# Duy1230/Map-Reduced-Approach-for-Vietnamese-Long-Document-Summarization

Measured on AMD Instinct MI355X. Metric: map-phase chunks/sec (2k-tok chunk, 256-tok summary) at 1/2/4/8 MI355X, higher is better.
Workload: dtype f16

## Files before the change

### include/mapsum.h

```cpp
#ifndef MAPSUM_H
#define MAPSUM_H

#include <stddef.h>
#include <stdint.h>

#ifdef __cplusplus
extern "C" {
#endif

#define MS_ABI_VERSION 3

#define MS_OK 0
#define MS_EIO -5
#define MS_ENOMEM -12
#define MS_EBUSY -16
#define MS_EINVAL -22
#define MS_ENOSPC -28

#define MS_FINISH_EOS 1
#define MS_FINISH_LENGTH 2
#define MS_FINISH_ERROR 3

#define MS_FLAG_IGNORE_EOS 1u

// ... 30 lines not shown
  int32_t eos_ids[8];
} ms_config;

typedef struct ms_result {
  uint64_t tag;
  const int32_t* ids;
  int32_t n_ids;
  int32_t finish_reason;
  int32_t n_prompt;
  int32_t _pad;
} ms_result;

typedef struct ms_stats {
  int64_t prefill_tokens;
  int64_t decode_tokens;
  int64_t prefill_passes, decode_steps;
  int64_t finished;
  double prefill_ms, decode_ms;
  double kernel_ms[8];
  int64_t kernel_launches[8];
  int64_t decode_kv_tokens;
  int64_t graphs_built;
  int64_t persist_fallbacks;
  int64_t persist_steps;
} ms_stats;

typedef struct ms_engine ms_engine;

int ms_create(const ms_config* cfg, ms_engine** out);
int ms_destroy(ms_engine* e);
const char* ms_last_error(const ms_engine* e);

int ms_enable_qk_norm(ms_engine* e);

int ms_load_weight(ms_engine* e, int32_t tensor, int32_t layer, const uint16_t* host_f16,
                   int64_t n_elems);
int ms_init_synthetic(ms_engine* e, uint64_t seed, float std, float norm_jitter);

#define MS_GGML_Q8_0 8
#define MS_GGML_Q4_K 12
#define MS_GGML_Q5_K 13
#define MS_GGML_Q6_K 14
int ms_load_weight_q(ms_engine* e, int32_t tensor, int32_t layer, int32_t ggml_type,
                     const void* host_blocks, int64_t n_bytes);
int ms_init_synthetic_q(ms_engine* e, uint64_t seed, float scale, float norm_jitter);
int ms_init_synthetic_q8_0(ms_engine* e, uint64_t seed, float scale, float norm_jitter);
int ms_init_synthetic_q5_k_m(ms_engine* e, uint64_t seed, float scale, float norm_jitter);

int ms_weight_regions(const ms_engine* e, void** ptrs, int64_t* bytes, int32_t cap);
int ms_quant_manifest(const ms_engine* e, int32_t* triples, int32_t cap);
int ms_declare_weight_q(ms_engine* e, int32_t tensor, int32_t layer, int32_t ggml_type);

int ms_submit(ms_engine* e, const int32_t* ids, int32_t n, int32_t num_predict,
              uint32_t flags, uint64_t tag);
#define MS_SAMPLE_MAX_TOPK 256
#define MS_SAMPLE_MAX_WINDOW 256
typedef struct ms_sampling {
  float temperature;
  int32_t top_k;
  float top_p;
  float min_p;
  float repeat_penalty;
  int32_t repeat_last_n;
  uint64_t seed;
} ms_sampling;
int ms_submit_sampled(ms_engine* e, const int32_t* ids, int32_t n, int32_t num_predict,
                      uint32_t flags, uint64_t tag, const ms_sampling* sp);
int ms_set_eos_ids(ms_engine* e, const int32_t* ids, int32_t n);
int ms_step(ms_engine* e);
int ms_poll(ms_engine* e, ms_result* out, int32_t cap);
int ms_pending(const ms_engine* e);
int ms_get_stats(const ms_engine* e, ms_stats* out);
int ms_reset_stats(ms_engine* e);
int ms_set_profiling(ms_engine* e, uint32_t class_mask);
int ms_trace_push(const char* name);
int ms_trace_pop(void);
int ms_synchronize(ms_engine* e);
int ms_set_persist(ms_engine* e, int32_t on);
#define MS_DBG_KPOOL 0
#define MS_DBG_VPOOL 1
#define MS_DBG_DECODE_LOGITS 2
#define MS_DBG_DECODE_X 3
#define MS_DBG_PREFILL_LOGITS 4
int ms_debug_read(ms_engine* e, int32_t which, int64_t offset, void* host, int64_t bytes);
int ms_debug_pk_stamps(uint64_t* out, int32_t n);
int ms_debug_a2_stamps(uint64_t* out, int32_t n);
int ms_debug_gemv_stamps(uint64_t* out, int32_t n);

int ms_forward(ms_engine* e, const int32_t* ids, int32_t n, int32_t n_layers_run,
               float* hidden_out, float* logits_out);
int ms_forward_packed(ms_engine* e, const int32_t* ids, const int32_t* lens, int32_t n_seqs,
                      int32_t n_layers_run, float* hidden_out, float* logits_out);
int ms_submit_forced(ms_engine* e, const int32_t* ids, int32_t n, const int32_t* forced,
                     int32_t n_forced, int32_t num_predict, uint32_t flags, uint64_t tag);

#define MS_EPI_STORE_F16 0
#define MS_EPI_ADD_F32 1
#define MS_EPI_SWIGLU 2
#define MS_EPI_STORE_F32 3
#define MS_EPI_ARGMAX 5
int ms_op_gemm(const void* A, const void* W, void* out, int32_t M, int32_t N, int32_t K,
               int32_t ldo, int32_t epilogue, void* stream);
int ms_op_gemm_resid(const void* A, const void* W, float* x, void* xg_out, const void* gamma, float* ssq_out,
                     int32_t M, int32_t N, int32_t K, void* stream);
int ms_gemm_resid_tiles(int32_t M, int32_t N);
int ms_set_gemm_variant(int32_t variant);
#define MS_GEMV_ORDER_DEFAULT (-1)
int ms_set_gemv_order(int32_t order);
int ms_set_qgemv_gs(int32_t on);
int ms_set_attn_tuning(int32_t combine_grp, int32_t order);
int ms_set_dgemm_kh(int32_t kh);
int ms_set_dgemm_wn(int32_t wn);
int64_t ms_op_gemv_workspace(int32_t M, int32_t N, int32_t K);
int ms_op_gemv(const void* X, const void* W, void* out, int32_t M, int32_t N, int32_t K,
               int32_t ldo, int32_t epilogue, void* workspace, void* stream);
int ms_op_gemv_tuned(const void* X, const void* W, void* out, int32_t M, int32_t N, int32_t K,
                     int32_t ldo, int32_t epilogue, void* workspace, int32_t waves, void* stream);
int ms_op_gemv_strided(const void* X, const void* W, void* out, int32_t M, int32_t N, int32_t K,
                       int32_t ldk, int32_t ldo, int32_t epilogue, void* stream);
int ms_op_gemv_resid(const void* X, const void* W, float* x, void* xg_out, const void* gamma,
                     float* ssq_out, int32_t M, int32_t N, int32_t K, int32_t rt, void* stream);
int ms_op_set_row_scale(const float* ssq, int32_t tiles, int32_t hidden, float eps);
int ms_op_dgemm(const void* X, const void* W, void* out, int32_t M, int32_t N, int32_t K, int32_t S,
                int32_t ldo, int32_t epilogue, void* stream);
int ms_op_gemv_split(const void* X, const void* W, float* slabs, int32_t M, int32_t N, int32_t K,
                     int32_t S, int32_t waves, void* stream);
int ms_op_residual_rmsnorm(float* x, const float* slabs, int32_t S, const void* w, void* y, float* ssq,
                           int32_t rows, int32_t hidden, void* stream);
int ms_op_dequant(int32_t ggml_type, const void* blocks, int64_t n_blocks, float* out, void* stream);
int ms_op_quant_rows(int32_t ggml_type, const void* blocks, int32_t rows, int32_t K, void* f16_out,
                     void* packed_out, void* stream);
int ms_op_qgemv(const void* X, int32_t ggml_type, const void* packed_rows, void* out, int32_t M,
                int32_t N, int32_t K, int32_t ldo, int32_t epilogue, void* stream);
int ms_op_qgemv_split(const void* X, int32_t ggml_type, const void* packed_rows, float* slabs,
                      int32_t M, int32_t N, int32_t K, int32_t S, void* stream);
int ms_op_qgemv_resid(const void* X, int32_t ggml_type, const void* packed_rows, float* x, void* xg_out,
                      const void* gamma, float* ssq_out, int32_t M, int32_t N, int32_t K, int32_t rt,
                      void* stream);
int ms_op_qdgemm(const void* X, int32_t ggml_type, const void* packed_rows, void* out, int32_t M,
                 int32_t N, int32_t K, int32_t S, int32_t ldo, int32_t epilogue, void* stream);
int ms_op_rmsnorm(const void* x, const void* w, void* y, float* ssq, int32_t rows, int32_t hidden,
                  const int32_t* row_idx, void* stream);
int ms_op_qk_norm_rope(void* qkv, const float* slabs, int32_t S, int32_t T, int32_t n_heads, int32_t n_kv_heads,
                       const int32_t* tok_pos, const int32_t* tok_slot, const float* cos_tab, const float* sin_tab,
                       const void* q_gain, const void* k_gain, float eps, void* k_pool, void* v_pool,
                       const int32_t* block_table, int32_t max_pages, void* stream);
int ms_op_argmax(const void* logits, int32_t rows, int32_t n, int32_t* ids, void* stream);
int ms_op_argmax_partials(const void* partials, int32_t rows, int32_t tiles, int32_t* ids, void* stream);
int ms_op_sample(const float* logits, int32_t rows, int32_t n, int64_t ldl, const ms_sampling* params,
                 const int32_t* win, const int32_t* win_len, const int32_t* steps, int32_t* ids,
                 int32_t* cand_ids, float* cand_p, int32_t* cand_n, void* stream);

#ifdef __cplusplus
}
#endif
#endif
```

### map-reduced-approach-for-vietnamese-long-document-summarization_amd/csrc/engine.cpp

```cpp
#include <hip/hip_runtime.h>

#include <algorithm>
#include <cmath>
#include <cstddef>
#include <cstdio>
#include <cstring>
#include <deque>
#include <array>
#include <map>
#include <tuple>
#include <memory>
#include <string>
#include <vector>

#if MS_HAVE_ROCTX
#include <rocprofiler-sdk-roctx/roctx.h>
#else
static inline int roctxRangePushA(const char*) { return 0; }
static inline int roctxRangePop() { return 0; }
#endif

#include "decode_forms.h"
#include "internal.h"

// ... 1553 lines not shown
        E.done.push_back(std::move(*it));
        it = E.running.erase(it);
      } else {
        ++it;
      }
    }
    return (int)(E.waiting.size() + E.running.size());
  });
}

int ms_poll(ms_engine* e, ms_result* out, int32_t cap) {
  if (!e) return MS_EINVAL;
  return guarded(e, [&]() -> int {
    ms_engine& E = *e;
    REQUIRE(cap >= 0 && (cap == 0 || out != nullptr), MS_EINVAL, "bad poll buffer");
    E.polled.clear();
    const int n = std::min<int>(cap, (int)E.done.size());
    for (int i = 0; i < n; ++i) {
      Seq& s = *E.done[i];
      out[i].tag = s.tag;
      out[i].ids = s.out.data();
      out[i].n_ids = (int32_t)s.out.size();
      out[i].finish_reason = s.finish;
      out[i].n_prompt = (int32_t)s.prompt.size();
      out[i]._pad = 0;
    }
    for (int i = 0; i < n; ++i) E.polled.push_back(std::move(E.done[i]));
    E.done.erase(E.done.begin(), E.done.begin() + n);
    return n;
  });
}

int ms_trace_push(const char* name) {
  if (!name) return MS_EINVAL;
  roctxRangePushA(name);
  return MS_OK;
}

int ms_trace_pop(void) {
  roctxRangePop();
  return MS_OK;
}

int ms_get_stats(const ms_engine* e, ms_stats* out) {
  if (!e || !out) return MS_EINVAL;
  *out = e->stats;
  return MS_OK;
}

int ms_reset_stats(ms_engine* e) {
  if (!e) return MS_EINVAL;
  e->stats = ms_stats{};
  return MS_OK;
}

int ms_set_profiling(ms_engine* e, uint32_t mask) {
  if (!e) return MS_EINVAL;
  e->prof_mask = mask;
  return MS_OK;
}

int ms_set_persist(ms_engine* e, int32_t on) {
  if (!e) return MS_EINVAL;
  return guarded(e, [&]() -> int {
    HIP_OK(hipStreamSynchronize(e->cd.stream));
    e->S.persist = on != 0;
    e->drop_graphs();
    return (e->persist_ok ? 1 : 0);
  });
}

int ms_debug_read(ms_engine* e, int32_t which, int64_t offset, void* host, int64_t bytes) {
  if (!e || !host || offset < 0 || bytes < 0) return MS_EINVAL;
  return guarded(e, [&]() -> int {
    ms_engine& E = *e;
    const void* base = nullptr;
    size_t cap = 0;
    switch (which) {
      case MS_DBG_KPOOL: base = E.kpool; cap = E.layer_kv_elems * E.L * sizeof(f16_t); break;
      case MS_DBG_VPOOL: base = E.vpool; cap = E.layer_kv_elems * E.L * sizeof(f16_t); break;
      case MS_DBG_DECODE_LOGITS: base = E.cd.logits; cap = (size_t)E.cfg.max_batch * E.V * sizeof(float); break;
      case MS_DBG_DECODE_X: base = E.cd.x; cap = (size_t)E.cfg.max_batch * E.H * sizeof(float); break;
      case MS_DBG_PREFILL_LOGITS: base = E.cp.logits; cap = (size_t)E.cfg.max_batch * E.V * sizeof(float); break;
      default: REQUIRE(false, MS_EINVAL, "ms_debug_read: unknown buffer");
    }
    REQUIRE((size_t)offset + (size_t)bytes <= cap, MS_EINVAL, "ms_debug_read: range past the buffer");
    HIP_OK(hipStreamSynchronize(E.cd.stream));
    HIP_OK(hipStreamSynchronize(E.cp.stream));
    HIP_OK(hipMemcpy(host, (const char*)base + offset, (size_t)bytes, hipMemcpyDeviceToHost));
    return MS_OK;
  });
}

int ms_synchronize(ms_engine* e) {
  if (!e) return MS_EINVAL;
  return guarded(e, [&]() -> int {
    HIP_OK(hipStreamSynchronize(e->cp.stream));
    HIP_OK(hipStreamSynchronize(e->cd.stream));
    return MS_OK;
  });
}

int ms_forward_packed(ms_engine* e, const int32_t* ids, const int32_t* lens, int32_t n_seqs,
                      int32_t n_layers_run, float* hidden_out, float* logits_out) {
  if (!e) return MS_EINVAL;
  return guarded(e, [&]() -> int {
    ms_engine& E = *e;
    HIP_OK(hipSetDevice(E.cfg.device));
    REQUIRE(E.waiting.empty() && E.running.empty(), MS_EBUSY, "ms_forward needs an idle engine");
    REQUIRE(ids && lens && n_seqs >= 1 && n_seqs <= (int)E.free_slots.size(), MS_EINVAL,
            "bad probe batch (1 <= n_seqs <= max_batch)");
    REQUIRE(n_layers_run >= 0 && n_layers_run <= E.L, MS_EINVAL, "n_layers_run out of range");
    REQUIRE(!logits_out || n_layers_run == E.L, MS_EINVAL, "logits need every layer");
    int64_t T = 0, pages = 0;
    for (int i = 0; i < n_seqs; ++i) {
      REQUIRE(lens[i] >= 1 && lens[i] <= E.cfg.max_ctx, MS_EINVAL, "bad probe length");
      T += lens[i];
      pages += (lens[i] + kPage - 1) / kPage;
    }
    REQUIRE(T <= E.cfg.max_prefill_tokens, MS_EINVAL, "probe longer than max_prefill_tokens");
    REQUIRE(pages <= (int64_t)E.free_pages.size(), MS_ENOSPC, "not enough KV pages");
    for (int64_t i = 0; i < T; ++i) REQUIRE(ids[i] >= 0 && ids[i] < E.V, MS_EINVAL, "token id out of range");
    E.use(E.cp);
    E.started = true;
    std::vector<Seq> seqs(n_seqs);
    std::vector<Seq*> b;
    int64_t off = 0;
    for (int i = 0; i < n_seqs; ++i) {
      seqs[i].prompt.assign(ids + off, ids + off + lens[i]);
      off += lens[i];
      reserve(E, seqs[i], lens[i]);
      b.push_back(&seqs[i]);
    }
    float* lg = nullptr;
    try {
      if (logits_out) HIP_OK(hipMalloc((void**)&lg, (size_t)T * E.V * sizeof(float)));
      prefill(E, b, n_layers_run, lg, nullptr);
      HIP_OK(hipStreamSynchronize(E.stream));
      if (hidden_out)
        HIP_OK(hipMemcpy(hidden_out, E.x, (size_t)T * E.H * sizeof(float), hipMemcpyDeviceToHost));
      if (logits_out)
        HIP_OK(hipMemcpy(logits_out, lg, (size_t)T * E.V * sizeof(float), hipMemcpyDeviceToHost));
    } catch (...) {
      if (lg) (void)hipFree(lg);
      for (Seq& s : seqs) release(E, s);
      throw;
    }
    if (lg) (void)hipFree(lg);
    for (Seq& s : seqs) release(E, s);
    E.ev_pending.clear();
    E.ev_used = 0;
    return MS_OK;
  });
}

int ms_forward(ms_engine* e, const int32_t* ids, int32_t n, int32_t n_layers_run, float* hidden_out,
               float* logits_out) {
  return ms_forward_packed(e, ids, &n, 1, n_layers_run, hidden_out, logits_out);
}

}
```

### map-reduced-approach-for-vietnamese-long-document-summarization_amd/csrc/k_attn.hip

```cpp
#include <algorithm>

#include "attn_common.h"

namespace ms {

template <int GB>
__global__ __launch_bounds__(512, 1) void attn_prefill_kernel(const f16_t* __restrict__ qkv,
                                                              f16_t* __restrict__ out, int Hq,
                                                              int Hk, KVView kv, PrefillAttnArgs a,
                                                              float scale_log2) {
  constexpr int QR = kPrefillQRows;
  __shared__ __attribute__((aligned(16))) char smem[2 * 32768 + GB * QR * 256];
  const int tid = threadIdx.x, lane = tid & 63, wave = tid >> 6;
  const int g = lane >> 4, r = lane & 15;
  const int ngrp = Hq / GB;
  const int e = a.qblk[blockIdx.x / ngrp];
  const int h0 = (blockIdx.x % ngrp) * GB;
  const int sq = e >> 16, qb = e & 0xFFFF;
  const int qlen = a.seq_qlen[sq], kvlen = a.seq_kvlen[sq], qstart = a.seq_qstart[sq];
  const int slot = a.seq_slot[sq];
  const int kvh = h0 / (Hq / Hk);
  const int row_stride = (Hq + 2 * Hk) * kHeadDim;
  const int q0 = qb * QR + wave * 16;
  const int qi = q0 + r;
// ... 542 lines not shown
}

static int g_combine_grp = [] { const char* e = getenv("MS_COMBINE_GRP"); return e ? atoi(e) : 1; }();
void set_attn_tuning(int combine_grp, int order) {
  (void)order;
  g_combine_grp = combine_grp;
}
static bool combine_grp_ok(int B, int Hk) { return g_combine_grp != 0 && (B * Hk) % 8 == 0; }

static void launch_combine(const float* ws, f16_t* out, int B, int Hq, int Hk, int nsplit, bool grp,
                           hipStream_t s) {
#define CB(P_)                                                                                          \
  do {                                                                                                  \
    if (grp)                                                                                            \
      MS_LAUNCH((attn_decode_combine_kernel<P_, true>), dim3(B * Hq), dim3(128), 0, s, ws, out, Hq,     \
                nsplit, Hk, B);                                                                         \
    else                                                                                                \
      MS_LAUNCH((attn_decode_combine_kernel<P_, false>), dim3(B, Hq), dim3(128), 0, s, ws, out, Hq,     \
                nsplit, Hk, B);                                                                         \
  } while (0)
  if (nsplit <= 4) CB(4);
  else if (nsplit <= 8) CB(8);
  else CB(16);
#undef CB
}

void launch_attn_decode(const DecodeQKV& qa, f16_t* out, int Hq, int Hk, KVView kv,
                        DecodeAttnArgs a, float* ws, hipStream_t s) {
  if (a.B <= 0) return;
  const int ppw = a.ppw > 0 ? a.ppw : 2;
  if (!attn_decode_supported(a.B, Hq, Hk, a.max_len, ppw)) return;
  if (qa.slabs && (qa.S < 1 || qa.S > kMaxSlabs)) return;
  if (qa.slabs && qa.rs.ssq && (qa.rs.tiles < 1 || qa.rs.tiles > 256)) return;
  const int nsplit = decode_nsplit(ppw, a.max_len);
  const float scale_log2 = kLog2e / sqrtf((float)kHeadDim);
  const dim3 grid(a.B, Hk, nsplit);
#define AD(SL)                                                                                              \
  do {                                                                                                      \
    if (ppw == 2)                                                                                           \
      MS_LAUNCH((attn_decode_kernel<SL, 2>), grid, dim3(256), 0, s, qa, Hq, Hk, kv, a, ws, nsplit, ppw,     \
                scale_log2);                                                                                \
    else                                                                                                    \
      MS_LAUNCH((attn_decode_kernel<SL, 0>), grid, dim3(256), 0, s, qa, Hq, Hk, kv, a, ws, nsplit, ppw,     \
                scale_log2);                                                                                \
  } while (0)
  if (qa.slabs) AD(true);
  else AD(false);
#undef AD
  launch_combine(ws, out, a.B, Hq, Hk, nsplit, false, s);
}

}

namespace ms {

constexpr int kPpbMin = 4, kPpbMax = 9;

int attn_decode2_ppb(int max_batch, int Hk, int max_ctx) {
  const char* ev = getenv("MS_ATTN_PPB");
  const int env = ev ? atoi(ev) : 0;
  if (env > 0) return std::max(kPpbMin, std::min(env, kPpbMax));
  const long np = (max_ctx + kPage - 1) / kPage;
  const long want = (np * max_batch * Hk + 255) / 256;
  return (int)std::max((long)kPpbMin, std::min((long)kPpbMax, want));
}

static size_t attn2_lds_bytes(int ppb, int G) {
  return (size_t)ppb * 16384 + (size_t)(G + 2) * kHeadDim * 4 + (size_t)(G + 2) * kHeadDim * 2 + 16;
}
bool attn_decode2_supported(int B, int Hq, int Hk, int max_len, int ppb) {
  (void)B;
  if (Hk < 1 || Hq % Hk || Hq / Hk > kMaxGroup || ppb < kPpbMin || ppb > kPpbMax) return false;
  const int np = (max_len + kPage - 1) / kPage;
  return (np + ppb - 1) / ppb <= kMaxSplits && attn2_lds_bytes(ppb, Hq / Hk) <= 160 * 1024;
}

size_t attn_decode2_workspace_bytes(int B, int Hq, int max_len, int ppb) {
  const int np = (max_len + kPage - 1) / kPage;
  return (size_t)B * Hq * ((np + ppb - 1) / ppb) * 132 * sizeof(float);
}

constexpr int kA2StampBlocks = 1024, kA2Stamps = 32;
__device__ unsigned long long g_a2_stamps[kA2StampBlocks * kA2Stamps];
#define A2_STAMP(k)                                                                               \
  do {                                                                                            \
    if (stamps && lane == 0 && blockIdx.x < kA2StampBlocks)                                       \
      stamps[blockIdx.x * kA2Stamps + (k)] = __builtin_amdgcn_s_memrealtime();                    \
  } while (0)

template <bool FROM_SLABS, int PPB, bool TICKET>
__global__ __launch_bounds__(64 * PPB) void attn_decode2_kernel(
    DecodeQKV qa, int Hq, int Hk, KVView kv, DecodeAttnArgs a, float* __restrict__ ws, f16_t* __restrict__ out,
    int nsplit, float scale_log2, unsigned* __restrict__ cnt, unsigned long long* __restrict__ stamps) {
  extern __shared__ __attribute__((aligned(16))) char smem[];
  constexpr int NTHR = 64 * PPB;
  const int tid = threadIdx.x, lane = tid & 63;
  const int wave = __builtin_amdgcn_readfirstlane(tid >> 6);
  const int g = lane >> 4, r = lane & 15;
  const int BH = a.B * Hk;
  const int split = blockIdx.x / BH, grp = blockIdx.x - split * BH;
  const int b = grp / Hk, kvh = grp - b * Hk;
  const int G = Hq / Hk;
  const int len = a.seq_len[b];
  const int slot = a.seq_slot[b];
  const int np = (len + kPage - 1) / kPage;
  const int pg = split * PPB + wave;
  const int pos = len - 1;
  const int row_stride = (Hq + 2 * Hk) * kHeadDim;
  char* vs_ = smem + wave * 16384;
  float* raw = (float*)(smem + (size_t)PPB * 16384);
  f16_t* qn = (f16_t*)(raw + (G + 2) * kHeadDim);
  f16_t* kn = qn + G * kHeadDim;
  f16_t* vn = kn + kHeadDim;
  const bool has_page = pg < np;
  if (wave == PPB - 1) A2_STAMP(24);
  if (stamps && wave == 0) {
    A2_STAMP(0);
    unsigned hw, xcc;
    asm volatile("s_getreg_b32 %0, hwreg(HW_REG_HW_ID)" : "=s"(hw));
    asm volatile("s_getreg_b32 %0, hwreg(HW_REG_XCC_ID)" : "=s"(xcc));
    if (lane == 0 && blockIdx.x < kA2StampBlocks)
      stamps[blockIdx.x * kA2Stamps + 1] = ((unsigned long long)xcc << 32) | hw;
  }
  const size_t pbase = (((size_t)slot * kv.max_pages + pg) * kv.n_kv_heads + kvh) * kPage * kHeadDim;

  const bool owns_new = (pos / kPage) / PPB == split;
  const int nvec = FROM_SLABS ? (G + (owns_new ? 2 : 0)) * kHeadDim : 0;
  constexpr int PER = ((kMaxGroup + 2) * kHeadDim + NTHR - 1) / NTHR;
  float rv[4] = {0.f, 0.f, 0.f, 0.f};
  float sv[PER][kMaxSlabs];
  float rcs = 0.f, rsn = 0.f;
  if constexpr (FROM_SLABS) {
    if (qa.rs.ssq) {
#pragma unroll
      for (int i = 0; i < 4; ++i) {
        const int t = lane + 64 * i;
        if (64 * i < qa.rs.tiles) rv[i] = ld_f32_opaque(qa.rs.ssq + (size_t)min(t, qa.rs.tiles - 1) * a.B + b);
      }
    }
    const size_t sstride = (size_t)a.B * row_stride;
    const float* src = qa.slabs + (size_t)b * row_stride;
#pragma unroll
    for (int i = 0; i < PER; ++i) {
      if (i * NTHR < nvec) {
        const int e = min(tid + i * NTHR, nvec - 1);
        const int hh = e >> 7, j = e & 127;
        const int col = hh < G ? (kvh * G + hh) * kHeadDim + j
                               : (hh == G ? (Hq + kvh) * kHeadDim + j : (Hq + Hk + kvh) * kHeadDim + j);
#pragma unroll
        for (int q = 0; q < kMaxSlabs; ++q)
          if (q < qa.S) sv[i][q] = ld_f32_opaque(src + q * sstride + col);
      }
    }
    rcs = ld_f32_opaque(qa.cos_tab + (size_t)pos * 64 + (tid & 63));
    rsn = ld_f32_opaque(qa.sin_tab + (size_t)pos * 64 + (tid & 63));
    if (wave == 0) A2_STAMP(26);
    if (wave == PPB - 1) A2_STAMP(25);
  }
  u32x4 kf[4][4];
  if (has_page) {
#pragma unroll
    for (int i = 0; i < 16; ++i) {
      const int rr = 4 * i + (lane >> 4), ch = (lane & 15) ^ ((rr & 7) << 1);
      dma16_opaque(kv.v + pbase + rr * kHeadDim + ch * 8, vs_ + i * 1024);
    }
#pragma unroll
// ... 51 lines not shown
                           kHeadDim + tid;
      kv.k[o] = kn[tid];
      kv.v[o] = vn[tid];
    }
  }
  if (wave == 0) A2_STAMP(2);

  f32x4 o[8];
#pragma unroll
  for (int i = 0; i < 8; ++i) o[i] = f32x4{0.f, 0.f, 0.f, 0.f};
  float m_run = -INFINITY, l_run = 0.f;
  if (has_page) {
    f16x8 qf[4];
    const int hl = min(r, G - 1);
    if constexpr (FROM_SLABS) {
#pragma unroll
      for (int s4 = 0; s4 < 4; ++s4) qf[s4] = *(const f16x8*)(qn + hl * kHeadDim + 32 * s4 + 8 * g);
    } else {
      const f16_t* qrow = qa.qkv + (size_t)b * row_stride + (kvh * G + hl) * kHeadDim;
#pragma unroll
      for (int s4 = 0; s4 < 4; ++s4) qf[s4] = as_f16x8(*(const uint4*)(qrow + 32 * s4 + 8 * g));
    }
    const int off = pos % kPage;
    const bool patch = FROM_SLABS && pg == pos / kPage;
    if (patch) {
#pragma unroll
      for (int mt = 0; mt < 4; ++mt)
#pragma unroll
        for (int s4 = 0; s4 < 4; ++s4)
          if (mt * 16 + r == off) kf[mt][s4] = *(const u32x4*)(kn + 32 * s4 + 8 * g);
    }
    f32x4 sc[4];
#pragma unroll
    for (int mt = 0; mt < 4; ++mt) {
      sc[mt] = f32x4{0.f, 0.f, 0.f, 0.f};
#pragma unroll
      for (int s4 = 0; s4 < 4; ++s4) sc[mt] = mfma16(__builtin_bit_cast(f16x8, kf[mt][s4]), qf[s4], sc[mt]);
    }
    float mx = -INFINITY;
#pragma unroll
    for (int mt = 0; mt < 4; ++mt)
#pragma unroll
      for (int j = 0; j < 4; ++j) {
        const int key = pg * kPage + mt * 16 + 4 * g + j;
        const float v = (key >= len) ? -INFINITY : sc[mt][j] * scale_log2;
        sc[mt][j] = v;
        mx = fmaxf(mx, v);
      }
    mx = grp_max(mx);
    A2_STAMP(3 + wave);
    float rs = 0.f;
#pragma unroll
    for (int mt = 0; mt < 4; ++mt)
#pragma unroll
      for (int j = 0; j < 4; ++j) {
        const float p = (sc[mt][j] == -INFINITY) ? 0.f : __builtin_amdgcn_exp2f(sc[mt][j] - mx);
        sc[mt][j] = p;
        rs += p;
      }
    l_run = grp_sum(rs);
    m_run = mx;
    wait_vmcnt0();
    if (pg == np - 1) {
      const int first = len - pg * kPage;
      for (int e = first * 16 + lane; e < 64 * 16; e += 64)
        *(u32x4*)(vs_ + v_swz(e >> 4, e & 15)) = u32x4{0, 0, 0, 0};
    }
    if (patch && lane < 16) *(u32x4*)(vs_ + v_swz(off, lane)) = *(const u32x4*)(vn + lane * 8);
    __builtin_amdgcn_s_waitcnt(0xC07F);
    __builtin_amdgcn_wave_barrier();
#pragma unroll
    for (int kstep = 0; kstep < 2; ++kstep) {
      const f16x8 pf = pack_p(sc[2 * kstep], sc[2 * kstep + 1]);
#pragma unroll
      for (int dt = 0; dt < 8; ++dt) {
        const f16x8 vt = load_vt(vs_, dt, kstep, lane);
        o[dt] = mfma16(vt, pf, o[dt]);
      }
    }
    __builtin_amdgcn_s_waitcnt(0xC07F);
    __builtin_amdgcn_wave_barrier();
    A2_STAMP(12 + wave);
  }
  {
    float* mw = (float*)vs_;
    if (g == 0) { mw[r * 130 + 0] = m_run; mw[r * 130 + 1] = l_run; }
#pragma unroll
    for (int dt = 0; dt < 8; ++dt)
#pragma unroll
      for (int j = 0; j < 4; ++j) mw[r * 130 + 2 + dt * 16 + 4 * g + j] = o[dt][j];
  }
  __syncthreads();
  for (int idx = tid; idx < G * 130; idx += NTHR) {
    const int c = idx / 130, k = idx - c * 130;
    float M = -INFINITY;
#pragma unroll
    for (int w = 0; w < PPB; ++w) M = fmaxf(M, ((const float*)(smem + w * 16384))[c * 130]);
    float acc = 0.f, L = 0.f;
#pragma unroll
    for (int w = 0; w < PPB; ++w) {
      const float* mw = (const float*)(smem + w * 16384);
      const float m_w = mw[c * 130];
      const float f = (m_w == -INFINITY) ? 0.f : __builtin_amdgcn_exp2f(m_w - M);
      acc += (k == 0) ? 0.f : f * mw[c * 130 + k];
      L += f * mw[c * 130 + 1];
    }
    if (nsplit == 1) {
      if (k >= 2) out[(size_t)b * Hq * kHeadDim + (kvh * G + c) * kHeadDim + (k - 2)] = f2h(acc / L);
    } else if constexpr (TICKET) {
      __hip_atomic_store(ws + (((size_t)b * Hq + kvh * G + c) * nsplit + split) * 132 + k, (k == 0) ? M : acc,
                         __ATOMIC_RELAXED, __HIP_MEMORY_SCOPE_AGENT);
    } else {
      ws[(((size_t)b * Hq + kvh * G + c) * nsplit + split) * 132 + k] = (k == 0) ? M : acc;
    }
  }
  if (stamps) {
    asm volatile("s_waitcnt vmcnt(0)" ::: "memory");
    if (wave == 0) A2_STAMP(21);
  }
  if constexpr (TICKET) {
    if (nsplit == 1) return;
    __shared__ unsigned last_s;
    asm volatile("s_waitcnt vmcnt(0)" ::: "memory");
    __syncthreads();
    if (tid == 0) {
      const unsigned old = __hip_atomic_fetch_add(cnt + grp, 1u, __ATOMIC_RELAXED, __HIP_MEMORY_SCOPE_AGENT);
      last_s = old == (unsigned)(nsplit - 1);
    }
    __syncthreads();
    if (!last_s) return;
    auto ld = [](const float* p) { return __hip_atomic_load(p, __ATOMIC_RELAXED, __HIP_MEMORY_SCOPE_AGENT); };
    for (int idx = tid; idx < G * kHeadDim; idx += NTHR) {
      const int c = idx >> 7, d = idx & 127;
      const float* p = ws + ((size_t)b * Hq + kvh * G + c) * nsplit * 132;
      float M = -INFINITY;
      for (int q = 0; q < nsplit; ++q) M = fmaxf(M, ld(p + q * 132));
      float L = 0.f, O = 0.f;
      for (int q = 0; q < nsplit; ++q) {
        const float m_q = ld(p + q * 132);
        const float f = m_q == -INFINITY ? 0.f : __builtin_amdgcn_exp2f(m_q - M);
        L += f * ld(p + q * 132 + 1);
        O += f * ld(p + q * 132 + 2 + d);
      }
      out[(size_t)b * Hq * kHeadDim + (kvh * G + c) * kHeadDim + d] = f2h(O / L);
    }
    if (tid == 0) __hip_atomic_store(cnt + grp, 0u, __ATOMIC_RELAXED, __HIP_MEMORY_SCOPE_AGENT);
  }
}

void launch_attn_decode2(const DecodeQKV& qa, f16_t* out, int Hq, int Hk, KVView kv, DecodeAttnArgs a,
                         float* ws, int ppb, hipStream_t s, unsigned* cnt) {
  if (a.B <= 0) return;
  if (!attn_decode2_supported(a.B, Hq, Hk, a.max_len, ppb) || !kv.slot_major) return;
  if (qa.slabs && (qa.S < 1 || qa.S > kMaxSlabs)) return;
  if (qa.slabs && qa.rs.ssq && (qa.rs.tiles < 1 || qa.rs.tiles > 256)) return;
  const int np = (a.max_len + kPage - 1) / kPage;
  const int nsplit = (np + ppb - 1) / ppb;
  const float scale_log2 = kLog2e / sqrtf((float)kHeadDim);
  const dim3 grid(a.B * Hk * nsplit);
  const size_t lds = attn2_lds_bytes(ppb, Hq / Hk);
  static unsigned long long* stamps = [] {
    const char* e = getenv("MS_A2_STAMPS");
    void* p = nullptr;
    if (e && atoi(e)) (void)hipGetSymbolAddress(&p, HIP_SYMBOL(g_a2_stamps));
    return (unsigned long long*)p;
  }();
#define A2(P_)                                                                                                \
  case P_:                                                                                                    \
    if (qa.slabs && cnt)                                                                                      \
      MS_LAUNCH((attn_decode2_kernel<true, P_, true>), grid, dim3(64 * P_), lds, s, qa, Hq, Hk, kv, a, ws,    \
                out, nsplit, scale_log2, cnt, stamps);                                                        \
    else if (qa.slabs)                                                                                        \
      MS_LAUNCH((attn_decode2_kernel<true, P_, false>), grid, dim3(64 * P_), lds, s, qa, Hq, Hk, kv, a, ws,   \
                out, nsplit, scale_log2, cnt, stamps);                                                        \
    else                                                                                                      \
      MS_LAUNCH((attn_decode2_kernel<false, P_, false>), grid, dim3(64 * P_), lds, s, qa, Hq, Hk, kv, a, ws,  \
                out, nsplit, scale_log2, cnt, stamps);                                                        \
    break;
  switch (ppb) {
    A2(4) A2(5) A2(6) A2(7) A2(8) A2(9)
    default: return;
  }
#undef A2
  if (nsplit > 1 && !(qa.slabs && cnt)) launch_combine(ws, out, a.B, Hq, Hk, nsplit, combine_grp_ok(a.B, Hk), s);
}

}

namespace ms {
void attn2_stamps(unsigned long long* host, int n) {
  n = std::min(n, kA2StampBlocks * kA2Stamps);
  (void)hipMemcpyFromSymbol(host, HIP_SYMBOL(g_a2_stamps), (size_t)n * sizeof(unsigned long long));
}

void launch_attn_combine(const float* ws, f16_t* out, int B, int Hq, int Hk, int nsplit, hipStream_t s) {
  if (B <= 0 || nsplit <= 1) return;
  launch_combine(ws, out, B, Hq, Hk, nsplit, combine_grp_ok(B, Hk), s);
}
}
```

### map-reduced-approach-for-vietnamese-long-document-summarization_amd/mapsum/_lib.py

```python
from __future__ import annotations

import ctypes as C
import os

_HERE = os.path.dirname(os.path.abspath(__file__))
LIB_PATH = os.environ.get("MAPSUM_LIB") or os.path.join(_HERE, "libmapsum.so")

MS_ABI_VERSION = 3
MS_OK, MS_EIO, MS_ENOMEM, MS_EBUSY, MS_EINVAL, MS_ENOSPC = 0, -5, -12, -16, -22, -28
MS_FINISH_EOS, MS_FINISH_LENGTH, MS_FINISH_ERROR = 1, 2, 3
MS_FLAG_IGNORE_EOS = 1
(MS_T_EMBED, MS_T_ATTN_NORM, MS_T_WQ, MS_T_WK, MS_T_WV, MS_T_WO, MS_T_FFN_NORM, MS_T_WGATE,
 MS_T_WUP, MS_T_WDOWN, MS_T_FINAL_NORM, MS_T_LM_HEAD, MS_T_Q_NORM, MS_T_K_NORM) = range(14)
MS_EPI_STORE_F16, MS_EPI_ADD_F32, MS_EPI_SWIGLU, MS_EPI_STORE_F32 = range(4)
MS_EPI_ARGMAX = 5
GEMM_DEFAULT = 4
GEMV_ORDER_DEFAULT = -1
MS_GGML_Q8_0, MS_GGML_Q4_K, MS_GGML_Q5_K, MS_GGML_Q6_K = 8, 12, 13, 14
K_GEMM, K_ATTN_PREFILL, K_GEMV, K_ATTN_DECODE, K_LMHEAD, K_MISC, K_PERSIST = range(7)
MS_DBG_KPOOL, MS_DBG_VPOOL, MS_DBG_DECODE_LOGITS, MS_DBG_DECODE_X, MS_DBG_PREFILL_LOGITS = range(5)
MS_SAMPLE_MAX_TOPK, MS_SAMPLE_MAX_WINDOW = 256, 256

EXPORTED = (
    "ms_create", "ms_destroy", "ms_last_error", "ms_load_weight", "ms_init_synthetic",
    "ms_load_weight_q", "ms_init_synthetic_q", "ms_init_synthetic_q8_0", "ms_init_synthetic_q5_k_m", "ms_op_dequant", "ms_op_quant_rows", "ms_op_qgemv", "ms_op_qgemv_split", "ms_op_qgemv_resid", "ms_op_qdgemm",
    "ms_submit", "ms_step", "ms_poll", "ms_pending", "ms_get_stats", "ms_reset_stats",
    "ms_set_profiling", "ms_synchronize", "ms_forward", "ms_op_gemm", "ms_op_gemv_workspace",
    "ms_op_gemv", "ms_op_gemv_tuned", "ms_op_gemv_split", "ms_op_dgemm", "ms_op_residual_rmsnorm", "ms_op_rmsnorm",
    "ms_op_argmax", "ms_op_argmax_partials", "ms_set_gemm_variant", "ms_set_qgemv_gs", "ms_set_attn_tuning", "ms_set_dgemm_kh", "ms_set_dgemm_wn",
    "ms_weight_regions", "ms_quant_manifest", "ms_declare_weight_q",
    "ms_forward_packed", "ms_submit_forced", "ms_set_eos_ids", "ms_op_gemv_strided",
    "ms_op_gemv_resid", "ms_op_set_row_scale", "ms_op_gemm_resid", "ms_gemm_resid_tiles",
    "ms_trace_push", "ms_trace_pop", "ms_debug_a2_stamps", "ms_set_persist", "ms_debug_read", "ms_debug_pk_stamps",
    "ms_submit_sampled", "ms_op_sample", "ms_set_gemv_order", "ms_debug_gemv_stamps",
    "ms_enable_qk_norm", "ms_op_qk_norm_rope",
)


class MsConfig(C.Structure):
    _fields_ = [("abi_version", C.c_int32),
                ("n_layers", C.c_int32), ("hidden", C.c_int32), ("n_heads", C.c_int32),
                ("n_kv_heads", C.c_int32), ("head_dim", C.c_int32), ("ffn", C.c_int32),
                ("vocab", C.c_int32),
                ("rope_theta", C.c_float), ("rope_factor", C.c_float),
                ("rope_low_freq_factor", C.c_float), ("rope_high_freq_factor", C.c_float),
                ("rope_orig_ctx", C.c_int32), ("norm_eps", C.c_float), ("tie_embeddings", C.c_int32),
                ("device", C.c_int32), ("max_batch", C.c_int32), ("max_ctx", C.c_int32),
                ("max_prefill_tokens", C.c_int32), ("n_pages", C.c_int32), ("n_eos", C.c_int32),
                ("eos_ids", C.c_int32 * 8)]


class MsSampling(C.Structure):
    _fields_ = [("temperature", C.c_float), ("top_k", C.c_int32), ("top_p", C.c_float),
                ("min_p", C.c_float), ("repeat_penalty", C.c_float), ("repeat_last_n", C.c_int32),
                ("seed", C.c_uint64)]


class MsResult(C.Structure):
    _fields_ = [("tag", C.c_uint64), ("ids", C.POINTER(C.c_int32)), ("n_ids", C.c_int32),
                ("finish_reason", C.c_int32), ("n_prompt", C.c_int32), ("_pad", C.c_int32)]


class MsStats(C.Structure):
    _fields_ = [("prefill_tokens", C.c_int64), ("decode_tokens", C.c_int64),
                ("prefill_passes", C.c_int64), ("decode_steps", C.c_int64), ("finished", C.c_int64),
                ("prefill_ms", C.c_double), ("decode_ms", C.c_double),
                ("kernel_ms", C.c_double * 8), ("kernel_launches", C.c_int64 * 8),
                ("decode_kv_tokens", C.c_int64), ("graphs_built", C.c_int64),
                ("persist_fallbacks", C.c_int64), ("persist_steps", C.c_int64)]


_lib = None


def load() -> C.CDLL:
    global _lib
    if _lib is not None:
        return _lib
    if not os.path.exists(LIB_PATH):
        raise RuntimeError(f"libmapsum.so not found at {LIB_PATH}; build it with "
                           f"`make -C csrc` or `python -c 'import __graft_entry__ as g; g.build()'`")
    _lib = load_at(LIB_PATH, bool(os.environ.get("MAPSUM_LIB")))
    return _lib


def load_at(path: str, ab: bool = True) -> C.CDLL:
    lib = C.CDLL(path)
    vp, i32, i64, u32, u64 = C.c_void_p, C.c_int32, C.c_int64, C.c_uint32, C.c_uint64
    pi32 = C.POINTER(C.c_int32)
    sig = {
        "ms_create": (i32, [C.POINTER(MsConfig), C.POINTER(vp)]),
        "ms_destroy": (i32, [vp]),
        "ms_last_error": (C.c_char_p, [vp]),
        "ms_load_weight": (i32, [vp, i32, i32, vp, i64]),
        "ms_init_synthetic": (i32, [vp, u64, C.c_float, C.c_float]),
        "ms_load_weight_q": (i32, [vp, i32, i32, i32, vp, i64]),
        "ms_init_synthetic_q": (i32, [vp, u64, C.c_float, C.c_float]),
        "ms_init_synthetic_q8_0": (i32, [vp, u64, C.c_float, C.c_float]),
        "ms_init_synthetic_q5_k_m": (i32, [vp, u64, C.c_float, C.c_float]),
        "ms_op_dequant": (i32, [i32, vp, i64, vp, vp]),
        "ms_op_quant_rows": (i32, [i32, vp, i32, i32, vp, vp, vp]),
        "ms_op_qgemv": (i32, [vp, i32, vp, vp, i32, i32, i32, i32, i32, vp]),
        "ms_op_qgemv_split": (i32, [vp, i32, vp, vp, i32, i32, i32, i32, vp]),
# ... 88 lines not shown
```

Baseline: 13.10.

## Vectorize in-kernel split-KV combine and enable ticket combine for non-slab decode path

The decode attention kernel now writes per-split partials as 16-byte vector stores with sc1 cache hints, and the last-arriving block reduces all splits using batched inline-asm vector loads of 8 splits at a time. Each thread handles four elements of the head dimension instead of one. The ticket-based in-kernel combine is also enabled whenever a counter buffer exists, not only on the slab path, so the separate combine kernel launch is skipped more often. A debug read of the attention counter buffer is added. This relies on hand-written asm with cache-coherence hints and an acquire fence whose correctness depends on hardware ordering.

Result: no change. 13.09 (-0.0%).

```diff
diff --git a/include/mapsum.h b/include/mapsum.h
--- a/include/mapsum.h
+++ b/include/mapsum.h
@@ -136,6 +136,7 @@
 #define MS_DBG_DECODE_LOGITS 2
 #define MS_DBG_DECODE_X 3
 #define MS_DBG_PREFILL_LOGITS 4
+#define MS_DBG_ATTN_CNT 5
 int ms_debug_read(ms_engine* e, int32_t which, int64_t offset, void* host, int64_t bytes);
 int ms_debug_pk_stamps(uint64_t* out, int32_t n);
 int ms_debug_a2_stamps(uint64_t* out, int32_t n);
diff --git a/map-reduced-approach-for-vietnamese-long-document-summarization_amd/csrc/engine.cpp b/map-reduced-approach-for-vietnamese-long-document-summarization_amd/csrc/engine.cpp
--- a/map-reduced-approach-for-vietnamese-long-document-summarization_amd/csrc/engine.cpp
+++ b/map-reduced-approach-for-vietnamese-long-document-summarization_amd/csrc/engine.cpp
@@ -1659,6 +1659,7 @@
       case MS_DBG_DECODE_LOGITS: base = E.cd.logits; cap = (size_t)E.cfg.max_batch * E.V * sizeof(float); break;
       case MS_DBG_DECODE_X: base = E.cd.x; cap = (size_t)E.cfg.max_batch * E.H * sizeof(float); break;
       case MS_DBG_PREFILL_LOGITS: base = E.cp.logits; cap = (size_t)E.cfg.max_batch * E.V * sizeof(float); break;
+      case MS_DBG_ATTN_CNT: base = E.attn_cnt; cap = (size_t)E.cfg.max_batch * E.Hk * sizeof(unsigned); break;
       default: REQUIRE(false, MS_EINVAL, "ms_debug_read: unknown buffer");
     }
     REQUIRE((size_t)offset + (size_t)bytes <= cap, MS_EINVAL, "ms_debug_read: range past the buffer");
diff --git a/map-reduced-approach-for-vietnamese-long-document-summarization_amd/csrc/k_attn.hip b/map-reduced-approach-for-vietnamese-long-document-summarization_amd/csrc/k_attn.hip
--- a/map-reduced-approach-for-vietnamese-long-document-summarization_amd/csrc/k_attn.hip
+++ b/map-reduced-approach-for-vietnamese-long-document-summarization_amd/csrc/k_attn.hip
@@ -648,6 +648,36 @@
 
 constexpr int kA2StampBlocks = 1024, kA2Stamps = 32;
 __device__ unsigned long long g_a2_stamps[kA2StampBlocks * kA2Stamps];
+constexpr bool a2_one_per_cu(int ppb) { return 2 * ppb * 16384 > 160 * 1024; }
+
+__device__ __forceinline__ void st16_sc1(float* p, f32x4 v) {
+  asm volatile("global_store_dwordx4 %0, %1, off sc1" ::"v"(p), "v"(v) : "memory");
+}
+__device__ __forceinline__ void a2_fetch8(const float* p, int n, int piece, f32x4 (&ml)[8], f32x4 (&ov)[8]) {
+  const float* po = p + 4 * piece;
+  asm volatile("s_cmp_lt_i32 %18, 1\n\ts_cbranch_scc1 .La2_landed_%=\n\t"
+               "global_load_dwordx4 %0, %16, off sc1\n\tglobal_load_dwordx4 %8, %17, off sc1\n\t"
+               "s_cmp_lt_i32 %18, 2\n\ts_cbranch_scc1 .La2_landed_%=\n\t"
+               "global_load_dwordx4 %1, %16, off offset:528 sc1\n\tglobal_load_dwordx4 %9, %17, off offset:528 sc1\n\t"
+               "s_cmp_lt_i32 %18, 3\n\ts_cbranch_scc1 .La2_landed_%=\n\t"
+               "global_load_dwordx4 %2, %16, off offset:1056 sc1\n\tglobal_load_dwordx4 %10, %17, off offset:1056 sc1\n\t"
+               "s_cmp_lt_i32 %18, 4\n\ts_cbranch_scc1 .La2_landed_%=\n\t"
+               "global_load_dwordx4 %3, %16, off offset:1584 sc1\n\tglobal_load_dwordx4 %11, %17, off offset:1584 sc1\n\t"
+               "s_cmp_lt_i32 %18, 5\n\ts_cbranch_scc1 .La2_landed_%=\n\t"
+               "global_load_dwordx4 %4, %16, off offset:2112 sc1\n\tglobal_load_dwordx4 %12, %17, off offset:2112 sc1\n\t"
+               "s_cmp_lt_i32 %18, 6\n\ts_cbranch_scc1 .La2_landed_%=\n\t"
+               "global_load_dwordx4 %5, %16, off offset:2640 sc1\n\tglobal_load_dwordx4 %13, %17, off offset:2640 sc1\n\t"
+               "s_cmp_lt_i32 %18, 7\n\ts_cbranch_scc1 .La2_landed_%=\n\t"
+               "global_load_dwordx4 %6, %16, off offset:3168 sc1\n\tglobal_load_dwordx4 %14, %17, off offset:3168 sc1\n\t"
+               "s_cmp_lt_i32 %18, 8\n\ts_cbranch_scc1 .La2_landed_%=\n\t"
+               "global_load_dwordx4 %7, %16, off offset:3696 sc1\n\tglobal_load_dwordx4 %15, %17, off offset:3696 sc1\n"
+               ".La2_landed_%=:\n\ts_waitcnt vmcnt(0)"
+               : "=&v"(ml[0]), "=&v"(ml[1]), "=&v"(ml[2]), "=&v"(ml[3]), "=&v"(ml[4]), "=&v"(ml[5]), "=&v"(ml[6]),
+                 "=&v"(ml[7]), "=&v"(ov[0]), "=&v"(ov[1]), "=&v"(ov[2]), "=&v"(ov[3]), "=&v"(ov[4]), "=&v"(ov[5]),
+                 "=&v"(ov[6]), "=&v"(ov[7])
+               : "v"(p), "v"(po), "s"(n)
+               : "memory", "scc");
+}
 #define A2_STAMP(k)                                                                               \
   do {                                                                                            \
     if (stamps && lane == 0 && blockIdx.x < kA2StampBlocks)                                       \
@@ -865,7 +895,7 @@
     __builtin_amdgcn_wave_barrier();
     A2_STAMP(12 + wave);
   }
-  {
+  if (r < G) {
     float* mw = (float*)vs_;
     if (g == 0) { mw[r * 130 + 0] = m_run; mw[r * 130 + 1] = l_run; }
 #pragma unroll
@@ -874,7 +904,8 @@
       for (int j = 0; j < 4; ++j) mw[r * 130 + 2 + dt * 16 + 4 * g + j] = o[dt][j];
   }
   __syncthreads();
-  for (int idx = tid; idx < G * 130; idx += NTHR) {
+  const bool wide = TICKET && nsplit > 1;
+  for (int idx = tid; idx < (wide ? 0 : G * 130); idx += NTHR) {
     const int c = idx / 130, k = idx - c * 130;
     float M = -INFINITY;
 #pragma unroll
@@ -890,11 +921,31 @@
     }
     if (nsplit == 1) {
       if (k >= 2) out[(size_t)b * Hq * kHeadDim + (kvh * G + c) * kHeadDim + (k - 2)] = f2h(acc / L);
-    } else if constexpr (TICKET) {
-      __hip_atomic_store(ws + (((size_t)b * Hq + kvh * G + c) * nsplit + split) * 132 + k, (k == 0) ? M : acc,
-                         __ATOMIC_RELAXED, __HIP_MEMORY_SCOPE_AGENT);
     } else {
       ws[(((size_t)b * Hq + kvh * G + c) * nsplit + split) * 132 + k] = (k == 0) ? M : acc;
+    }
+  }
+  if constexpr (TICKET) {
+    for (int idx = tid; idx < (wide ? G * 33 : 0); idx += NTHR) {
+      const int c = idx / 33, j = idx - c * 33;
+      float M = -INFINITY;
+#pragma unroll
+      for (int w = 0; w < PPB; ++w) M = fmaxf(M, ((const float*)(smem + w * 16384))[c * 130]);
+      float acc[4] = {0.f, 0.f, 0.f, 0.f};
+#pragma unroll
+      for (int w = 0; w < PPB; ++w) {
+        const float* mw = (const float*)(smem + w * 16384);
+        const float m_w = mw[c * 130];
+        const float f = (m_w == -INFINITY) ? 0.f : __builtin_amdgcn_exp2f(m_w - M);
+#pragma unroll
+        for (int i = 0; i < 4; ++i) {
+          const int k = 4 * j + i;
+          const float t = (k == 0 || k >= 130) ? 0.f : __fmul_rn(f, mw[c * 130 + min(k, 129)]);
+          acc[i] = __fadd_rn(acc[i], t);
+        }
+      }
+      st16_sc1(ws + (((size_t)b * Hq + kvh * G + c) * nsplit + split) * 132 + 4 * j,
+               f32x4{j == 0 ? M : acc[0], acc[1], acc[2], acc[3]});
     }
   }
   if (stamps) {
@@ -908,24 +959,56 @@
     __syncthreads();
     if (tid == 0) {
       const unsigned old = __hip_atomic_fetch_add(cnt + grp, 1u, __ATOMIC_RELAXED, __HIP_MEMORY_SCOPE_AGENT);
-      last_s = old == (unsigned)(nsplit - 1);
+      const bool last = old == (unsigned)(nsplit - 1);
+      if constexpr (!a2_one_per_cu(PPB)) {
+        if (last) {
+          __builtin_amdgcn_fence(__ATOMIC_ACQUIRE, "agent");
+          asm volatile("s_waitcnt vmcnt(0)" ::: "memory");
+        }
+      }
+      last_s = last;
+      A2_STAMP(27);
     }
     __syncthreads();
     if (!last_s) return;
-    auto ld = [](const float* p) { return __hip_atomic_load(p, __ATOMIC_RELAXED, __HIP_MEMORY_SCOPE_AGENT); };
-    for (int idx = tid; idx < G * kHeadDim; idx += NTHR) {
-      const int c = idx >> 7, d = idx & 127;
+    for (int idx = tid; idx < G * 33; idx += NTHR) {
+      const int c = idx / 33, j = idx - c * 33;
       const float* p = ws + ((size_t)b * Hq + kvh * G + c) * nsplit * 132;
+      f32x4 ml[8], ov[8];
+      a2_fetch8(p, nsplit, j, ml, ov);
+      if (wave == 0) A2_STAMP(28);
       float M = -INFINITY;
-      for (int q = 0; q < nsplit; ++q) M = fmaxf(M, ld(p + q * 132));
-      float L = 0.f, O = 0.f;
-      for (int q = 0; q < nsplit; ++q) {
-        const float m_q = ld(p + q * 132);
-        const float f = m_q == -INFINITY ? 0.f : __builtin_amdgcn_exp2f(m_q - M);
-        L += f * ld(p + q * 132 + 1);
-        O += f * ld(p + q * 132 + 2 + d);
-      }
-      out[(size_t)b * Hq * kHeadDim + (kvh * G + c) * kHeadDim + d] = f2h(O / L);
+#pragma unroll
+      for (int q = 0; q < 8; ++q)
+        if (q < nsplit) M = fmaxf(M, ml[q][0]);
+      for (int base = 8; base < nsplit; base += 8) {
+        f32x4 m2[8], o2[8];
+        a2_fetch8(p + (size_t)base * 132, nsplit - base, 0, m2, o2);
+#pragma unroll
+        for (int q = 0; q < 8; ++q)
+          if (base + q < nsplit) M = fmaxf(M, m2[q][0]);
+      }
+      float L = 0.f, O[4] = {0.f, 0.f, 0.f, 0.f};
+      for (int base = 0; base < nsplit; base += 8) {
+        if (base > 0) a2_fetch8(p + (size_t)base * 132, nsplit - base, j, ml, ov);
+#pragma unroll
+        for (int q = 0; q < 8; ++q) {
+          if (base + q < nsplit) {
+            const float m_q = ml[q][0];
+            const float f = m_q == -INFINITY ? 0.f : __builtin_amdgcn_exp2f(m_q - M);
+            L = __fmaf_rn(f, ml[q][1], L);
+#pragma unroll
+            for (int i = 0; i < 4; ++i) O[i] = __fmaf_rn(f, ov[q][i], O[i]);
+          }
+        }
+      }
+      f16_t* o = out + (size_t)b * Hq * kHeadDim + (kvh * G + c) * kHeadDim + 4 * j;
+      if (j > 0) *(uint32_t*)(o - 2) = (uint32_t)f2h(O[0] / L) | ((uint32_t)f2h(O[1] / L) << 16);
+      if (j < 32) *(uint32_t*)o = (uint32_t)f2h(O[2] / L) | ((uint32_t)f2h(O[3] / L) << 16);
+    }
+    if (stamps) {
+      asm volatile("s_waitcnt vmcnt(0)" ::: "memory");
+      if (wave == 0) A2_STAMP(29);
     }
     if (tid == 0) __hip_atomic_store(cnt + grp, 0u, __ATOMIC_RELAXED, __HIP_MEMORY_SCOPE_AGENT);
   }
@@ -948,24 +1031,23 @@
     if (e && atoi(e)) (void)hipGetSymbolAddress(&p, HIP_SYMBOL(g_a2_stamps));
     return (unsigned long long*)p;
   }();
-#define A2(P_)                                                                                                \
-  case P_:                                                                                                    \
-    if (qa.slabs && cnt)                                                                                      \
-      MS_LAUNCH((attn_decode2_kernel<true, P_, true>), grid, dim3(64 * P_), lds, s, qa, Hq, Hk, kv, a, ws,    \
-                out, nsplit, scale_log2, cnt, stamps);                                                        \
-    else if (qa.slabs)                                                                                        \
-      MS_LAUNCH((attn_decode2_kernel<true, P_, false>), grid, dim3(64 * P_), lds, s, qa, Hq, Hk, kv, a, ws,   \
-                out, nsplit, scale_log2, cnt, stamps);                                                        \
-    else                                                                                                      \
-      MS_LAUNCH((attn_decode2_kernel<false, P_, false>), grid, dim3(64 * P_), lds, s, qa, Hq, Hk, kv, a, ws,  \
-                out, nsplit, scale_log2, cnt, stamps);                                                        \
+#define A2K(SL_, P_, T_)                                                                                      \
+  MS_LAUNCH((attn_decode2_kernel<SL_, P_, T_>), grid, dim3(64 * P_), lds, s, qa, Hq, Hk, kv, a, ws, out, nsplit, \
+            scale_log2, cnt, stamps)
+#define A2(P_)                                \
+  case P_:                                    \
+    if (qa.slabs && cnt) A2K(true, P_, true); \
+    else if (qa.slabs) A2K(true, P_, false);  \
+    else if (cnt) A2K(false, P_, true);       \
+    else A2K(false, P_, false);               \
     break;
   switch (ppb) {
     A2(4) A2(5) A2(6) A2(7) A2(8) A2(9)
     default: return;
   }
+#undef A2K
 #undef A2
-  if (nsplit > 1 && !(qa.slabs && cnt)) launch_combine(ws, out, a.B, Hq, Hk, nsplit, combine_grp_ok(a.B, Hk), s);
+  if (nsplit > 1 && !cnt) launch_combine(ws, out, a.B, Hq, Hk, nsplit, combine_grp_ok(a.B, Hk), s);
 }
 
 }
diff --git a/map-reduced-approach-for-vietnamese-long-document-summarization_amd/mapsum/_lib.py b/map-reduced-approach-for-vietnamese-long-document-summarization_amd/mapsum/_lib.py
--- a/map-reduced-approach-for-vietnamese-long-document-summarization_amd/mapsum/_lib.py
+++ b/map-reduced-approach-for-vietnamese-long-document-summarization_amd/mapsum/_lib.py
@@ -18,7 +18,7 @@
 GEMV_ORDER_DEFAULT = -1
 MS_GGML_Q8_0, MS_GGML_Q4_K, MS_GGML_Q5_K, MS_GGML_Q6_K = 8, 12, 13, 14
 K_GEMM, K_ATTN_PREFILL, K_GEMV, K_ATTN_DECODE, K_LMHEAD, K_MISC, K_PERSIST = range(7)
-MS_DBG_KPOOL, MS_DBG_VPOOL, MS_DBG_DECODE_LOGITS, MS_DBG_DECODE_X, MS_DBG_PREFILL_LOGITS = range(5)
+MS_DBG_KPOOL, MS_DBG_VPOOL, MS_DBG_DECODE_LOGITS, MS_DBG_DECODE_X, MS_DBG_PREFILL_LOGITS, MS_DBG_ATTN_CNT = range(6)
 MS_SAMPLE_MAX_TOPK, MS_SAMPLE_MAX_WINDOW = 256, 256
 
 EXPORTED = (
```
